# ajzhai/PEANUT

Measured on AMD Instinct MI355X. Metric: maps/sec for 480x480x(4+N_cat) prediction fwd, batch 32, higher is better.
Workload: dtype f32; 1 GPU; 480x480, 14-channel (4+10) partial maps -> 6-class prediction forward (PSPNet R50-V1c-D8), batch 32 per GPU, seeded random-init weights; survey_config=2, global_batch=32, parallelism=dp1 (map shards, no data-path collective)

## Files before the change

### peanut_amd/csrc/common.h

```cpp
#pragma once
#include <hip/hip_runtime.h>
#include <stdint.h>
#include <string>

#include "persistent_plan.h"

namespace peanut {

void set_error(const std::string& msg);
int fail(int code, const std::string& msg);
void note_kernel(const char* family);
const char* noted_kernel();

#define PEANUT_HIP_CHECK(expr)                                                            \
  do {                                                                                    \
    hipError_t _e = (expr);                                                               \
    if (_e != hipSuccess)                                                                 \
      return ::peanut::fail(-3, std::string(#expr) + ": " + hipGetErrorString(_e));       \
  } while (0)

struct ConvDesc {
  int cin;
  int cout;
  int kh, kw, stride, pad, dil;
  int relu;
  int bn_tile;
  int bk;
  int cout_pad;
  const float* w_packed;
  const float* scale;
  const float* shift;
  int rs;
  const void* w_s;
  int s_planes;
  float s_alpha;
  int flush_ch;
};

struct DeferredSplit {
  bool valid;
  const float* partial;
  int split_p, ntiles, M, cout, relu;
  const float* scale;
  const float* shift;
  float alpha;
};

struct ConvArgs {
  const float* x;
  const float* x2;
  const float* res;
  float* y;
  int B, H, W;
  int c1, c2;
  int Ho, Wo;
  float* ws;
  size_t ws_floats;
  int mt_per_group;
  size_t w_group_stride;
  int ss_group_stride;
  int group_valid_rows;
  DeferredSplit* defer;
  const int* group_rows;
};

constexpr size_t kSplitKScratchFloats = (size_t)48 << 20;
constexpr size_t kSplitKSideFloats = (size_t)8 << 20;

#if defined(__HIP_DEVICE_COMPILE__)
#define PEANUT_NO_PK_F32 __attribute__((target("no-packed-fp32-ops")))
#else
#define PEANUT_NO_PK_F32
#endif

__device__ __forceinline__ float paste_value(const float* __restrict__ m, int M, const float* __restrict__ bx, int x, int y) {
#pragma clang fp contract(off)
  const float gx = ((float)x + 0.5f - bx[0]) / (bx[2] - bx[0]) * 2.f - 1.f;
  const float gy = ((float)y + 0.5f - bx[1]) / (bx[3] - bx[1]) * 2.f - 1.f;
  const float ix = ((gx + 1.f) * (float)M - 1.f) / 2.f, iy = ((gy + 1.f) * (float)M - 1.f) / 2.f;
  const float fx = floorf(ix), fy = floorf(iy);
  const int x0 = (int)fminf(fmaxf(fx, -2.f), (float)M + 1.f), y0 = (int)fminf(fmaxf(fy, -2.f), (float)M + 1.f);
  if (x0 < -1 || x0 >= M || y0 < -1 || y0 >= M) return 0.f;
  const float lx = ix - fx, ly = iy - fy;
  const float wx = 1.f - lx, wy = 1.f - ly;
  auto at = [&](int yy, int xx) -> float {
    return ((unsigned)yy < (unsigned)M && (unsigned)xx < (unsigned)M) ? m[yy * M + xx] : 0.f;
  };
  return at(y0, x0) * wy * wx + at(y0, x0 + 1) * wy * lx + at(y0 + 1, x0) * ly * wx + at(y0 + 1, x0 + 1) * ly * lx;
}

inline int conv_out_dim(int n, int k, int s, int p, int d) { return (n + 2 * p - d * (k - 1) - 1) / s + 1; }

void conv_pick_tiles(int cin_pad, int cout, int* bn_tile, int* bk, bool pointwise = false);
size_t conv_packed_floats(int cin_pad, int cout, int kh, int kw, int bn_tile);
void pack_conv_weights(const float* w_oihw, int cout, int cin_real, int cin_pad, int kh, int kw,
                       int bn_tile, int bk, float* out);
int launch_conv(const ConvDesc& d, const ConvArgs& a, hipStream_t stream);

enum ConvKernelId {
  CONV_K_INVALID,
  CONV_K_GEMM_RS,
  CONV_K_CONV_RS,
  CONV_K_GEMM_SKINNY,
  CONV_K_PW_256X256P,
  CONV_K_PW_ARES,
  CONV_K_PW_256X256,
  CONV_K_PW_256X128P,
  CONV_K_PW_256X128,
  CONV_K_PW_TILE,
  CONV_K_PATCH,
  CONV_K_PATCH_NCHW,
  CONV_K_IGEMM,
};
struct ConvRoute {
  ConvKernelId id;
  int bm, bn, bk;
  int planes;
  int stride;
  int pack_bn;
  int G;
  PersistentPlan plan;
  int code;
  const char* error;
};
struct ConvKParams;
ConvRoute conv_route(const ConvDesc& d, const ConvArgs& a, ConvKParams* params = nullptr);
ConvRoute conv_route_patch_nchw();
const char* conv_kernel_family(const ConvRoute& r);
int device_cus();
bool conv_pw_enabled();
bool conv_pw_uses_256(int cout, long long M, int mt_per_group, int bn_tile, int cin);
int conv_pw_256_min_k();
bool conv_pw_uses_256w(int cout, long long M, int mt_per_group, int bn_tile, int cin, int flush_ktiles);
bool conv_pw_narrow_tiles(int cin, int cout, long long M, int bn_tile, int mt_per_group);
bool conv_pw_uses_256p(int cout, long long M, int mt_per_group, int bn_tile, int cin, int flush_ktiles, long long in_pixels = 0);
bool gemm_skinny_takes(const ConvKParams& p, int bn_tile, size_t ws_floats);
bool conv_pw_uses_256wp(int cout, long long M, int stride, int mt_per_group, int bn_tile, int c1, int c2, int flush_ktiles);
bool conv_pw_uses_ares(int cin, int cout, long long M, int stride, bool two_source, int flush_ktiles, int bn_tile);

bool conv_patch_eligible(const ConvDesc& d, const ConvArgs& a);
bool conv_patch_nchw_eligible(const ConvDesc& d, int B, int Ho, int Wo, int creal);
int launch_conv_patch_nchw(const ConvDesc& d, const float* x_nchw, int creal, float* y, int B, int H, int W, int Ho, int Wo, hipStream_t stream);

void wino_geometry(int B, int H, int W, int dil, int* th, int* tw, long long* n_tiles, long long* m_pad, int gran = 128, int m = 4);
void wino_transform_weights(const float* w_oihw, int cout, int cin, float* out, int m = 4);
int launch_wino_input(const float* x, float* V, int B, int H, int W, int C, int dil, hipStream_t s, int gran = 128, int m = 4, long long m_pad_total = 0,
                      const DeferredSplit* df = nullptr);
bool wino_input_accepts_deferred(int B, int H, int W, int C, int dil, int gran, int m);
long long wino_deferred_count();
int launch_wino_output(const float* Mb, const float* scale, const float* shift, const float* res, float* y,
                       int B, int H, int W, int C, int dil, int relu, hipStream_t s, int gran = 128, int m = 4, long long m_pad_total = 0);

bool gemm_rs_uses_256(int cout, long long M, int mt_per_group, int bn_tile, int cin);
bool gemm_rs_uses_64(int cout, long long M, int bn_tile, int cin);
size_t sx_packed_bytes(int cin_pad, int cout, int bn_tile, int planes);
void pack_weights_sx(const float* w, int cout, int cin_real, int cin_pad, int bn_tile, int planes, float wscale, void* out);
float sx_pack_scale(const float* w, size_t n, int planes);
size_t sx_conv_packed_bytes(int cin_pad, int cout, int kh, int kw, int bn_tile, int planes);
void pack_weights_sx_conv(const float* w_oihw, int cout, int cin_real, int cin_pad, int kh, int kw, int bn_tile, int planes,
                          float wscale, void* out);

int launch_nchw_to_nhwc_pad(const float* x, float* y, int B, int C, int H, int W, int Cpad, hipStream_t s);
int launch_maxpool3x3s2(const float* x, float* y, int B, int H, int W, int C, int Ho, int Wo, hipStream_t s);
int launch_ppm_pool(const float* x, float* out, int B, int H, int W, int C, const int* scales, int nscales,
                    hipStream_t s, int scale_rows = 0);
size_t ppm_pool_scratch_floats(int B, int H, int C, const int* scales, int nscales);
int launch_ppm_pool2(const float* x, float* scratch, float* out, int B, int H, int W, int C, const int* scales,
                     int nscales, hipStream_t s, int scale_rows = 0);
int launch_ppm_upsample_concat(const float* table, float* out, int B, int H, int W, int Cp, const int* scales,
                               int nscales, int align_corners, hipStream_t s);
int launch_ppm_conv_term(const float* Q, float* R, int B, int H, int W, int C, const int* scales, int nscales,
                         int align_corners, hipStream_t s, int scale_rows = 0);
int launch_upsample_logits(const float* lo, float* out, int B, int h, int w, int K, int H, int W,
                           int align_corners, int sigmoid, hipStream_t s);

}
```

### peanut_amd/csrc/conv_common.h

```cpp
#pragma once
#include <stdlib.h>

#include <atomic>

#include "common.h"
#include "options.h"

namespace peanut {

typedef float f32x16 __attribute__((ext_vector_type(16)));
typedef float f32x4 __attribute__((ext_vector_type(4)));

__device__ __forceinline__ float relu_keep_nan(float v) { return v < 0.f ? 0.f : v; }
__device__ __forceinline__ f32x4 relu_keep_nan(f32x4 v) {
  return f32x4{relu_keep_nan(v.x), relu_keep_nan(v.y), relu_keep_nan(v.z), relu_keep_nan(v.w)};
}

struct ConvKParams {
  const float* x;
  const float* x2;
  const float* w;
  const float* scale;
  const float* shift;
  const float* res;
  const float* zeros;
  float* y;
  int H, W, c1, c2, Ho, Wo, cout;
  int kw, ntaps, stride, pad, dil, relu;
  int M, nkt, ntiles, HoWo;
  int n_full, n_sp, split_p;
  float* partial;
  int mt_per_group;
  long long w_group_stride;
  int ss_group_stride;
  int mtiles;
  int nchunk;
  int res_prefetch;
  float alpha;
  int ares_pbn;
  int phase_shift;
  int sk_units, sk_maxp, sk_g, sk_q;
  int pack_bn;
  int group_valid;
  int p_order;
  float* dump;
  int stagger;
  int flush;
  DeferredSplit* defer;
  const int* group_rows;
};

template <int I>
struct IC { static constexpr int value = I; };
template <int N, int I = 0, class F>
__device__ __forceinline__ void static_for(F&& f) {
  if constexpr (I < N) {
    f(IC<I>{});
    static_for<N, I + 1>(f);
  }
}

struct KIter {
  int tap, ky, kx, cbase;
  const float* wtile;
};


const float* zero_page();
int launch_conv_pw(const ConvKParams& p, const ConvRoute& r, float* ws, size_t ws_floats, hipStream_t stream);
int launch_gemm_skinny(const ConvKParams& p, float* ws, size_t ws_floats, hipStream_t stream);
int launch_conv_pw_ares(const ConvKParams& p, int bn_tile, hipStream_t stream);
int launch_conv_pw256p(const ConvKParams& p, const ConvRoute& r, float* ws, hipStream_t stream);
int launch_conv_pw256wp(const ConvKParams& p, const ConvRoute& r, float* ws, hipStream_t stream);
int launch_conv_patch(const ConvKParams& p, const ConvDesc& d, int B, hipStream_t stream);
int launch_gemm_rs(const ConvKParams& p, const ConvRoute& r, int bn_tile, float* ws, size_t ws_floats, hipStream_t stream);
int launch_conv_rs(const ConvKParams& p, int bn_tile, int planes, float* ws, size_t ws_floats, hipStream_t stream);
int launch_conv_igemm(const ConvKParams& p, int bn_tile, int bk, float* ws, size_t ws_floats, hipStream_t stream);


struct Work { int mt, nt, kt0, kt1, item; };

__host__ __device__ __forceinline__ int sk_owner(long long U, int G, long long u) {
  int w = (int)(u * G / U);
  while (w + 1 < G && U * (w + 1) / G <= u) ++w;
  while (w > 0 && U * w / G > u) --w;
  return w;
}

__device__ __forceinline__ void tile_to_mn(const ConvKParams& p, int tile, int* mt_out, int* nt_out) {
  int mt, nt;
  if (p.nchunk > 0 && p.ntiles > p.nchunk) {
    const int full = p.ntiles / p.nchunk, rem = p.ntiles - full * p.nchunk;
    const int per_chunk = p.mtiles * p.nchunk;
    if (tile < full * per_chunk) {
      const int c = tile / per_chunk, r = tile - c * per_chunk;
      mt = r / p.nchunk;
      nt = c * p.nchunk + (r - mt * p.nchunk);
    } else {
      const int r = tile - full * per_chunk;
      mt = r / rem;
      nt = full * p.nchunk + (r - mt * rem);
    }
  } else {
    mt = tile / p.ntiles;
    nt = tile - mt * p.ntiles;
  }
  *mt_out = mt;
  *nt_out = nt;
}

__device__ __forceinline__ Work decode_work(const ConvKParams& p) {
  const int G = gridDim.x, bid = blockIdx.x;
  const int q = G >> 3, r = G & 7, xcd = bid & 7, local = bid >> 3;
  const int sq = p.n_sp >> 3, sr = p.n_sp & 7;
  const int sp_x = sq + (xcd < sr), sp_before = xcd * sq + (xcd < sr ? xcd : sr);
  const int chunk_before = xcd * q + (xcd < r ? xcd : r);
  Work w;
  int tile;
  if (local < sp_x) {
    const int s = sp_before + local;
    const int j = s / p.split_p, part = s - j * p.split_p;
    tile = p.n_full + j;
    w.item = s;
    w.kt0 = (int)((long long)part * p.nkt / p.split_p);
    w.kt1 = (int)((long long)(part + 1) * p.nkt / p.split_p);
  } else {
    tile = (chunk_before - sp_before) + (local - sp_x);
    w.item = -1;
    w.kt0 = 0;
    w.kt1 = p.nkt;
  }
  tile_to_mn(p, tile, &w.mt, &w.nt);
  return w;
}

constexpr int kResPrefetchRows = 8;
struct ResPrefetch { f32x4 v[kResPrefetchRows]; bool on; };

template <int BM, int BN, int EP, int NT>
__device__ __forceinline__ ResPrefetch conv_res_prefetch(const ConvKParams& p, const Work& wk, int m0, int n0) {
  constexpr int NV = BN / 4, ROWS_PER_PASS = NT / NV, ER = BM / EP;
  const int tid = threadIdx.x;
  const int c4 = (tid % NV) * 4, r0 = tid / NV, n = n0 + c4;
  ResPrefetch r;
  r.on = p.res_prefetch && p.res && wk.item < 0 && (p.cout & 3) == 0 && n < p.cout;
  if (r.on) {
#pragma unroll
    for (int i = 0; i < kResPrefetchRows; ++i) {
      const int row = r0 + i * ROWS_PER_PASS, m = m0 + row;
      r.v[i] = (row < ER && m < p.M) ? *reinterpret_cast<const f32x4*>(p.res + (size_t)m * p.cout + n) : f32x4{0.f, 0.f, 0.f, 0.f};
    }
  }
  return r;
}

template <int BM, int BN, int WM, int WN, int EP, int NT = 256, int MI = 0, int NI = 0>
__device__ __forceinline__ void conv_epilogue(const ConvKParams& p, const Work& wk, f32x16 (&acc)[MI][NI], float* smem,
                                              int m0, int n0, const ResPrefetch* early = nullptr) {
  constexpr int TM = BM / WM, TN = BN / WN;
  constexpr int CS = BN + 4, ER = BM / EP;
  static_assert(MI == TM / 32 && NI == TN / 32, "accumulator shape");
  const int tid = threadIdx.x;
  const int lane = tid & 63, wave = tid >> 6;
  const int wm = wave / WN, wn = wave % WN;
  const int li = lane & 31, hi = lane >> 5;
  constexpr int NV = BN / 4;
  constexpr int ROWS_PER_PASS = NT / NV;
  const int c4 = (tid % NV) * 4, r0 = tid / NV;
  const int n = n0 + c4;
  const int ss_off = (p.mt_per_group && p.ss_group_stride) ? (wk.mt / p.mt_per_group) * p.ss_group_stride : 0;
  const f32x4 sc = *reinterpret_cast<const f32x4*>(p.scale + ss_off + n) * p.alpha;
  const f32x4 sh = *reinterpret_cast<const f32x4*>(p.shift + ss_off + n);
  const bool vec_ok = (p.cout & 3) == 0;
  constexpr int PRE = kResPrefetchRows;
  const ResPrefetch rp = early ? *early : conv_res_prefetch<BM, BN, EP, NT>(p, wk, m0, n0);
  const f32x4 (&rpre)[PRE] = rp.v;
  const bool pre = rp.on;
#pragma unroll
  for (int ep = 0; ep < EP; ++ep) {
    if (EP == 1 || wm == ep) {
#pragma unroll
      for (int t = 0; t < MI; ++t)
#pragma unroll
        for (int u = 0; u < NI; ++u)
#pragma unroll
          for (int r = 0; r < 16; ++r) {
            const int row = wm * TM + t * 32 + (r & 3) + 8 * (r >> 2) + 4 * hi - ep * ER;
            smem[row * CS + wn * TN + u * 32 + li] = acc[t][u][r];
          }
    }
    __syncthreads();
    if (wk.item >= 0) {
      float* dst = p.partial + (size_t)wk.item * (BM * BN) + (size_t)ep * ER * BN;
      for (int row = r0; row < ER; row += ROWS_PER_PASS)
        *reinterpret_cast<f32x4*>(dst + row * BN + c4) = *reinterpret_cast<const f32x4*>(smem + row * CS + c4);
    } else {
      int row_first = r0;
      if (pre && ep == 0) {
#pragma unroll
        for (int i = 0; i < PRE; ++i) {
          const int row = r0 + i * ROWS_PER_PASS, m = m0 + row;
          if (row < ER && m < p.M) {
            f32x4 v = *reinterpret_cast<const f32x4*>(smem + row * CS + c4);
            v = v * sc + sh;
            v += rpre[i];
            if (p.relu) v = relu_keep_nan(v);
            const size_t o = (size_t)m * p.cout + n;
            *reinterpret_cast<f32x4*>(p.y + o) = v;
          }
        }
        row_first = r0 + PRE * ROWS_PER_PASS;
      }
#pragma unroll 4
      for (int row = row_first; row < ER; row += ROWS_PER_PASS) {
        const int m = m0 + ep * ER + row;
        if (m >= p.M) break;
        f32x4 v = *reinterpret_cast<const f32x4*>(smem + row * CS + c4);
        v = v * sc + sh;
        const size_t o = (size_t)m * p.cout + n;
        if (vec_ok) {
          if (n < p.cout) {
            if (p.res) v += *reinterpret_cast<const f32x4*>(p.res + o);
            if (p.relu) v = relu_keep_nan(v);
            *reinterpret_cast<f32x4*>(p.y + o) = v;
// ... 174 lines not shown
```

### peanut_amd/csrc/conv_route.hip

```cpp
#include "common.h"
#include "conv_common.h"
#include "rs_common.h"

namespace peanut {

int device_cus() {
  static std::atomic<int> cached[SlotCache::kMaxDevices];
  int dev = 0;
  if (hipGetDevice(&dev) != hipSuccess || dev < 0) return 0;
  const bool in_cache = dev < SlotCache::kMaxDevices;
  int cus = in_cache ? cached[dev].load(std::memory_order_relaxed) : 0;
  if (cus == 0) {
    if (hipDeviceGetAttribute(&cus, hipDeviceAttributeMultiprocessorCount, dev) != hipSuccess) return 0;
    if (in_cache) cached[dev].store(cus, std::memory_order_relaxed);
  }
  return cus;
}

namespace {

ConvRoute route_of(ConvKernelId id, int bm = 0, int bn = 0, int bk = 0) {
  ConvRoute r{};
  r.id = id; r.bm = bm; r.bn = bn; r.bk = bk;
  return r;
}
ConvRoute no_route(int code, const char* why) {
  ConvRoute r{};
  r.id = CONV_K_INVALID; r.code = code; r.error = why;
  return r;
}

ConvRoute route_pw(const ConvKParams& p, int bn_tile, size_t ws_floats) {
  if (gemm_skinny_takes(p, bn_tile, ws_floats)) return route_of(CONV_K_GEMM_SKINNY);
  const bool streamk = opt(OPT_PW256P_STREAMK) != 0;
  if (conv_pw_uses_256wp(p.cout, p.M, p.stride, p.mt_per_group, bn_tile, p.c1, p.c2, p.flush)) {
    const int cus = device_cus();
    if (cus < 8) return no_route(-3, "conv_pw256wp: no current device");
    ConvRoute r = route_of(CONV_K_PW_256X256P, 256, 256, 32);
    r.G = cus - cus % 8;
    r.plan = plan_persistent((p.M / 256) * (p.cout / 256), r.G, p.nkt, kPersistent256x256, streamk, ws_floats);
    if (r.plan.fits) return r;
  }
  if (conv_pw_uses_ares(p.c1, p.cout, p.M, p.stride, p.c2 != 0, p.flush, bn_tile)) return route_of(CONV_K_PW_ARES, 128, 128, 32);
  if (conv_pw_uses_256w(p.cout, p.M, p.mt_per_group, bn_tile, p.c1 + p.c2, p.flush)) return route_of(CONV_K_PW_256X256, 256, 256, 32);
  if (conv_pw_uses_256p(p.cout, p.M, p.mt_per_group, bn_tile, p.c1 + p.c2, p.flush, (long long)(p.M / p.HoWo) * p.H * p.W) && !(p.flush && p.res)) {
    const int cus = device_cus();
    if (cus < 8) return no_route(-3, "conv_pw256p: no current device");
    ConvRoute r = route_of(CONV_K_PW_256X128P, 256, 128, 32);
    r.G = cus - cus % 8;
    r.plan = plan_persistent(((p.M + 255) / 256) * p.ntiles, r.G, p.nkt, p.flush ? kPersistent256x128Flush : kPersistent256x128, streamk, ws_floats);
    if (r.plan.fits || !r.plan.scratch_ok) return r;
  }
  if (conv_pw_uses_256(p.cout, p.M, p.mt_per_group, bn_tile, p.c1 + p.c2)) return route_of(CONV_K_PW_256X128, 256, 128, 32);
  if (conv_pw_narrow_tiles(p.c1 + p.c2, p.cout, p.M, bn_tile, p.mt_per_group)) {
    ConvRoute r = route_of(CONV_K_PW_TILE, 128, 64, 32);
    r.pack_bn = 128;
    return r;
  }
  if (bn_tile != 128 && bn_tile != 64 && bn_tile != 32) return no_route(-2, "launch_conv_pw: unsupported tile configuration");
  return route_of(CONV_K_PW_TILE, 128, bn_tile, 32);
}

}

ConvRoute conv_route(const ConvDesc& d, const ConvArgs& a, ConvKParams* params) {
  if (a.c1 + a.c2 != d.cin) return no_route(-2, "launch_conv: c1 + c2 != cin");
  const bool rs_fallback = d.rs == 1 && a.c2 != 0 && d.stride != 1;
  const bool emulated = d.rs && !rs_fallback;
  const int kgran = emulated ? 16 : d.bk;
  if (a.c1 % kgran != 0 || (a.c2 % kgran) != 0) return no_route(-2, "launch_conv: channel split not a multiple of the k-tile");
  ConvKParams local;
  ConvKParams& p = params ? *params : local;
  p = ConvKParams{};
  p.x = a.x; p.x2 = a.x2 ? a.x2 : a.x; p.w = d.w_packed; p.scale = d.scale; p.shift = d.shift;
  p.res = a.res; p.y = a.y;
  p.H = a.H; p.W = a.W; p.c1 = a.c1; p.c2 = a.c2; p.Ho = a.Ho; p.Wo = a.Wo; p.cout = d.cout;
  p.kw = d.kw; p.ntaps = d.kh * d.kw; p.stride = d.stride; p.pad = d.pad; p.dil = d.dil; p.relu = d.relu;
  p.HoWo = a.Ho * a.Wo;
  const long long M = (long long)a.B * p.HoWo;
  if (M <= 0 || M > 0x7fffffffLL || (long long)a.B * a.H * a.W > 0x7fffffffLL)
    return no_route(-2, "launch_conv: problem size out of range");
  p.M = (int)M;
  p.nkt = (d.cin / d.bk) * p.ntaps;
  p.ntiles = d.cout_pad / d.bn_tile;
  p.n_full = 0; p.n_sp = 0; p.split_p = 1; p.partial = nullptr;
  p.alpha = 1.f;
  p.flush = emulated ? 0 : d.flush_ch / d.bk;
  p.mt_per_group = a.mt_per_group; p.w_group_stride = (long long)a.w_group_stride; p.ss_group_stride = a.ss_group_stride;
  p.group_valid = a.mt_per_group ? a.group_valid_rows : 0;
  p.defer = a.defer;
  p.group_rows = a.mt_per_group ? a.group_rows : nullptr;
  if (emulated) {
    p.w = static_cast<const float*>(d.w_s);
    p.nkt = (d.cin / 16) * p.ntaps;
    p.alpha = d.s_alpha;
    ConvRoute r = route_of(CONV_K_CONV_RS, 128, d.bn_tile, 16);
    if (d.rs != 2) {
      const int cin = p.c1 + p.c2;
      if (gemm_rs_uses_64(p.cout, p.M, d.bn_tile, cin)) r = route_of(CONV_K_GEMM_RS, 64, 64, 16);
      else if (gemm_rs_uses_256(p.cout, p.M, p.mt_per_group, d.bn_tile, cin)) r = route_of(CONV_K_GEMM_RS, 256, 256, 16);
      else r = route_of(CONV_K_GEMM_RS, 128, d.bn_tile == 128 ? 128 : 64, 16);
    }
    r.planes = d.s_planes;
    return r;
  }
  if (d.bk == 32 && p.ntaps == 1 && p.pad == 0 && p.c1 % 32 == 0 && p.c2 % 32 == 0 && (p.c2 == 0 || p.stride == 1) && conv_pw_enabled())
    return route_pw(p, d.bn_tile, a.ws ? a.ws_floats : 0);
  if (conv_patch_eligible(d, a)) {
    ConvRoute r = route_of(CONV_K_PATCH, 0, d.cout, d.cin);
    r.stride = d.stride;
    return r;
  }
  if ((d.bk != 32 && d.bk != 16) || (d.bn_tile != 128 && d.bn_tile != 64 && d.bn_tile != 32))
    return no_route(-2, "launch_conv: unsupported tile configuration");
  return route_of(CONV_K_IGEMM, 128, d.bn_tile, d.bk);
}

int launch_conv(const ConvDesc& d, const ConvArgs& a, hipStream_t stream) {
  ConvKParams p;
  const ConvRoute r = conv_route(d, a, &p);
  if (r.id == CONV_K_INVALID) return fail(r.code, r.error);
  p.zeros = zero_page();
  if (!p.zeros) return fail(-3, "launch_conv: zero page allocation failed");
  if (a.defer) a.defer->valid = false;
  if ((r.id == CONV_K_GEMM_RS || r.id == CONV_K_CONV_RS) && !d.w_s) return fail(-2, "launch_conv: register-split layer without pre-split weights");
  note_kernel(conv_kernel_family(r));
  switch (r.id) {
    case CONV_K_GEMM_RS: return launch_gemm_rs(p, r, d.bn_tile, a.ws, a.ws_floats, stream);
    case CONV_K_CONV_RS: return launch_conv_rs(p, d.bn_tile, d.s_planes, a.ws, a.ws_floats, stream);
    case CONV_K_GEMM_SKINNY: return launch_gemm_skinny(p, a.ws, a.ws_floats, stream);
    case CONV_K_PW_256X256P: return launch_conv_pw256wp(p, r, a.ws, stream);
    case CONV_K_PW_ARES: return launch_conv_pw_ares(p, d.bn_tile, stream);
    case CONV_K_PW_256X128P: return launch_conv_pw256p(p, r, a.ws, stream);
    case CONV_K_PW_256X256:
    case CONV_K_PW_256X128:
    case CONV_K_PW_TILE: return launch_conv_pw(p, r, a.ws, a.ws_floats, stream);
    case CONV_K_PATCH: return launch_conv_patch(p, d, a.B, stream);
    case CONV_K_IGEMM: return launch_conv_igemm(p, d.bn_tile, d.bk, a.ws, a.ws_floats, stream);
    case CONV_K_PATCH_NCHW:
    case CONV_K_INVALID: break;
  }
  return fail(-2, "launch_conv: no kernel");
}

ConvRoute conv_route_patch_nchw() {
  ConvRoute r = route_of(CONV_K_PATCH_NCHW, 0, 32, 16);
  r.stride = 2;
  return r;
}

const char* conv_kernel_family(const ConvRoute& r) {
  const int ni = r.bn == 128 ? 0 : (r.bn == 64 ? 1 : 2);
  const int kind = r.planes - RS_BF16X3;
  switch (r.id) {
    case CONV_K_INVALID: break;
    case CONV_K_IGEMM: {
      static const char* const names[2][3] = {{"conv_igemm_128x128x32", "conv_igemm_128x64x32", "conv_igemm_128x32x32"},
                                              {"conv_igemm_128x128x16", "conv_igemm_128x64x16", "conv_igemm_128x32x16"}};
      return names[r.bk == 32 ? 0 : 1][ni];
    }
    case CONV_K_CONV_RS: {
      static const char* const names[3][3] = {{"conv_rs3_128x128", "conv_rs3_128x64", "conv_rs3_128x32"},
                                              {"conv_rs6_128x128", "conv_rs6_128x64", "conv_rs6_128x32"},
                                              {"conv_rs3h_128x128", "conv_rs3h_128x64", "conv_rs3h_128x32"}};
      return kind < 0 || kind > 2 ? "conv_rs?" : names[kind][ni];
    }
    case CONV_K_GEMM_RS: {
      static const char* const names[3][4] = {{"gemm_rs3_64x64", "gemm_rs3_256x256", "gemm_rs3_128x128", "gemm_rs3_128x64"},
                                              {"gemm_rs6_64x64", "gemm_rs6_256x256", "gemm_rs6_128x128", "gemm_rs6_128x64"},
                                              {"gemm_rs3h_64x64", "gemm_rs3h_256x256", "gemm_rs3h_128x128", "gemm_rs3h_128x64"}};
      return kind < 0 || kind > 2 ? "gemm_rs?" : names[kind][r.bm == 64 ? 0 : (r.bm == 256 ? 1 : (r.bn == 128 ? 2 : 3))];
    }
    case CONV_K_GEMM_SKINNY: return "gemm_skinny";
    case CONV_K_PW_256X256P: return "conv_pw_glds_256x256p";
    case CONV_K_PW_ARES: return "conv_pw_ares_128x128";
    case CONV_K_PW_256X256: return "conv_pw_glds_256x256";
    case CONV_K_PW_256X128P: return "conv_pw_glds_256x128p";
    case CONV_K_PW_256X128: return "conv_pw_glds_256x128";
    case CONV_K_PW_TILE: return ni == 0 ? "conv_pw_glds_128x128" : (ni == 1 ? "conv_pw_glds_128x64" : "conv_pw_glds_128x32");
    case CONV_K_PATCH:
      if (r.bk == 32) return r.bn == 64 ? "conv_patch_32x64s1" : "conv_patch_32x32s1";
      return r.stride == 1 ? "conv_patch_16x32s1" : "conv_patch_16x32s2";
    case CONV_K_PATCH_NCHW: return "conv_patch_nchw_16x32s2";
  }
  return "none";
}

}
```

### peanut_amd/csrc/options.h

```cpp
#pragma once
#include <stdlib.h>
#include <string.h>

#include <string>

namespace peanut {

enum OptionId {
  OPT_PW_GLDS, OPT_PW256_MINK, OPT_PW256_MINTILES, OPT_PW256_PHASE, OPT_PW256_SKIP_PAD, OPT_PW256W_MINK, OPT_PW256W_MINTILES, OPT_PW256P_MINK, OPT_PW256P_MINTILES, OPT_PW256P_FLUSH, OPT_PW256P_ORDER, OPT_PW256P_STREAMK, OPT_PW256WP_MINK, OPT_PW256WP_MINTILES, OPT_PW256WP_NPRE, OPT_PW256WP_STAGGER, OPT_PW_ARES, OPT_PW_SKINNY,
  OPT_PW_ARES_MINUNITS, OPT_PATCH_MINTILES, OPT_STEM_NCHW, OPT_BN64_MAXK, OPT_PW_BN64_MAXK, OPT_PW64_MAXTILES, OPT_FP32_BK, OPT_NCHUNK, OPT_RES_PREFETCH, OPT_SPLIT_MODEL,
  OPT_RS_CONV, OPT_RS_BN64_MAXK, OPT_RS256_MINK, OPT_RS256_MINTILES, OPT_RS64_MAXK, OPT_RS64_MAXTILES,
  OPT_WINO_M, OPT_WINO_HEAD_M, OPT_WINO6_MAXDIL, OPT_WINO5_MINDIL, OPT_WINO_FLUSH_CH, OPT_WINO_MIN_CIN, OPT_WINO_NARROW_MINPIX, OPT_WINO_SMALL_MAXWG, OPT_DEFER_SPLITK,
  OPT_PPM_OVERLAP, OPT_PPM_GROUPED, OPT_PPM_TERM_ROWS, OPT_PPM_GROUP_ROWS, OPT_RCNN_WINO_M, OPT_RCNN_STEM_S2D, OPT_RCNN_RPN_FUSED, OPT_RCNN_FPN_OVERLAP, OPT_RCNN_RANK_SORT, OPT_RCNN_TOPK_SLICE, OPT_RCNN_NMS_LEVELS, OPT_FMM_LOCAL32, OPT_FMM_MAX_PASSES, OPT_FMM_BLOCKED, OPT_FMM_INNER,
  OPT_DEBUG_POISON_ALLOC,
  OPT_COUNT
};

struct OptionInfo {
  const char* key;
  long long def;
  bool upload_time;
  const char* help;
};

inline const OptionInfo* option_table() {
  static const OptionInfo t[OPT_COUNT] = {
      {"pw_glds", 1, false, "fp32 1x1 convs / grouped GEMMs on the LDS-DMA kernels of conv_pw.hip (0: conv_igemm)"},
      {"pw256_mink", 1024, false, "fewest input channels for the 256 x 128 three-stage kernel"},
      {"pw256_mintiles", 256, false, "fewest 256 x 128 tiles for that kernel"},
      {"pw256_phase", 1, false, "the two waves of a SIMD request their LDS-DMA pieces half an iteration apart"},
      {"pw256_skip_pad", 1, false, "256 x 128 kernel, grouped GEMMs: waves whose rows are all group padding issue no MFMAs (0: compute the zero rows)"},
      {"pw256w_mink", 768, false, "fewest input channels for the 256 x 256 two-stage kernel (0: off)"},
      {"pw256w_mintiles", 1536, false, "fewest 256 x 256 tiles for that kernel"},
      {"pw256p_mink", 512, false, "fewest input channels for the persistent 256 x 128 kernel (conv_pw256p.hip; 0: off)"},
      {"pw256p_mintiles", 512, false, "fewest 256 x 128 tiles for that kernel"},
      {"pw256p_flush", 512, false, "most input channels of a Winograd position GEMM (two-level accumulation) that runs on the persistent kernel (0: none)"},
      {"pw256p_order", 1, false, "persistent 256 x 128 kernel: 1 = the workgroups of an XCD walk its run of tiles side by side (neighbours share operand panels in L2), 0 = one contiguous run per workgroup"},
      {"pw256p_streamk", 1, false, "persistent 256 x 128 kernel: the tail tiles' k-tiles as one stream in equal runs per workgroup (0: every tail tile cut into the same number of parts)"},
      {"pw256wp_mink", 512, false, "fewest input channels for the persistent 256 x 256 kernel (conv_pw256wp.hip; 0: off)"},
      {"pw256wp_mintiles", 768, false, "fewest 256 x 256 tiles for that kernel"},
      {"pw256wp_npre", 0, false, "persistent 256 x 256 kernel: accumulator blocks per in-place epilogue group (2 or 4; 0 = two with a residual, four without)"},
      {"pw256wp_stagger", 0, false, "persistent 256 x 256 kernel: spread of the workgroups' start times in sleeps of ~3.4 us (their tile boundaries -- 512 KiB of epilogue traffic per CU -- then fall at different times)"},
      {"pw_ares", 1, false, "K = 128 / 256 pointwise layers on the persistent A-resident kernel (conv_pw_ares.hip)"},
      {"pw_skinny", 1, false, "grouped pointwise launches with at most 64 data rows per group (the PSP pyramid's per-scale convs and Q tables at batch 1) on the skinny weight-streaming kernel (gemm_skinny.hip: 6 KiB of LDS, fits next to any other kernel; 0: the MFMA kernels on 128-row padded tiles)"},
      {"pw_ares_minunits", 512, false, "fewest (m-tile, n-tile) units for that kernel"},
      {"patch_mintiles", 1024, false, "3x3 convs of 16 / 32 input channels on the persistent LDS-patch kernel (conv_patch.hip) from this many 8 x 16 output tiles (0: off)"},
      {"stem_nchw", 1, false, "prediction forward: the first stem conv reads the NCHW input itself (conv_patch.hip, NCHW variant) instead of a layout pass + NHWC conv (fp32 mode, when the patch kernel takes the layer)"},
      {"bn64_maxk", 256, true, "128 x 64 tiles for layers with at most this many input channels"},
      {"pw_bn64_maxk", 128, true, "pointwise layers / Winograd position GEMMs: weights PACKED 64 wide up to this many input channels (wider layers: 128-wide packing, 64-wide tiles chosen per shape)"},
      {"pw64_maxtiles", 512, false, "a 128-wide-packed pointwise layer with at most bn64_maxk input channels runs 128 x 64 tiles while its 128 x 128 tiling has fewer tiles than this (two per CU)"},
      {"fp32_bk", 0, true, "16: force 16-channel k-tiles in conv_igemm (experiment)"},
      {"nchunk", 8, false, "n-tiles per chunk of the tile order (0: n fastest over all n-tiles)"},
      {"res_prefetch", 1, false, "request the first residual rows before the last k-tile's MFMAs"},
      {"split_model", 1, false, "tail split-K plan counts CUs (1) or resident slots (0)"},
      {"rs_conv", 1, true, "emulated modes: non-pointwise convs on conv_rs.hip (0: fp32 MFMA kernel)"},
      {"rs_bn64_maxk", 128, true, "emulated modes: 128 x 64 tiles up to this many input channels"},
      {"rs256_mink", 512, false, "emulated modes: fewest input channels for the 256 x 256 kernel"},
      {"rs256_mintiles", 256, false, "emulated modes: fewest 256 x 256 tiles for it"},
      {"rs64_maxk", 512, false, "emulated modes: 64 x 64 tiles up to this many input channels"},
      {"rs64_maxtiles", 128, false, "emulated modes: ... and below this many 128-row tiles"},
      {"wino_m", 0, true, "4 / 5 / 6: force one Winograd form on every eligible layer (0: policy)"},
      {"wino_head_m", 0, true, "4 / 5 / 6: Winograd form of the PSP bottleneck (0: policy)"},
      {"wino6_maxdil", 4, true, "largest dilation that gets an F(6x6) form"},
      {"wino5_mindil", 4, true, "smallest dilation that also gets an F(5x5) form (0: none)"},
      {"wino_flush_ch", 64, true, "channels per partial sum of the position GEMMs' two-level accumulation (0: off)"},
      {"wino_min_cin", 0, true, "fewest input channels of a Winograd layer (0: the planner's policy)"},
      {"wino_narrow_minpix", 20000, false, "layers under 128 channels take their Winograd form from this many input pixels on (round 6: 100 000 -> 20 000 -- with the small-problem transforms one 720 x 720 map's layer1 conv2, 32 400 pixels, gains 5 us per layer as F(6x6); profiles/r9e)"},
      {"wino_small_maxwg", 1024, false, "Winograd transforms: launches with fewer workgroups than this of the one-thread-per-tile kernels take the small-problem variants (a workgroup per tile and 64-channel slice, a thread per line, through LDS; bit-identical; 0: never)"},
      {"defer_splitk", 1, false, "a Bottleneck conv1 whose every tile is split along k leaves its partial tiles unsummed and conv2's (small-problem) Winograd input transform sums them: one launch fewer per block at batch 1, bit-identical (0: every conv runs its own reduce); read when a (B, H, W) plan is built"},
      {"ppm_overlap", -1, false, "pyramid branch of the PSP head on a side stream: 0 / 1, -1 = by size"},
      {"ppm_grouped", -1, false, "per-scale PSP GEMMs as one grouped launch: 0 / 1, -1 = by size"},
      {"ppm_term_rows", 1, false, "folded pyramid term: one wave per output row, no barrier in the row loop (0: the workgroup-wide two-phase kernel)"},
      {"ppm_group_rows", 0, false, "pyramid pooling, row pass: rows added up per workgroup (1..5; 0 = by size: as many as still leave ~768 workgroups)"},
      {"rcnn_wino_m", 0, true, "detector front end: 4 / 5 / 6 pins one Winograd form (0: per shape)"},
      {"rcnn_stem_s2d", 1, true, "detector stem 7x7 stride 2 as a space-to-depth 4x4 conv"},
      {"rcnn_rpn_fused", 1, false, "detector: the RPN head on all five pyramid levels as one chain (five input transforms, ONE grouped Winograd GEMM, five output transforms, one objectness and one anchor-delta GEMM over all levels' rows: 12 launches instead of 25); read when a (B, H, W) plan is built"},
      {"rcnn_fpn_overlap", 0, false, "detector: the FPN output convs of p5, p4, p3 on a side stream next to the lateral / top-down chain that ends in p2's (round 5 experiment, bit-identical; measured SLOWER at batch 1, 5.70 against 5.61 ms per frame, profiles/r8: off); read when a (B, H, W) plan is built"},
      {"rcnn_rank_sort", 1, false, "detector: the RPN candidates of an image are ordered by counting the larger keys (n / 64 workgroups) instead of one workgroup's bitonic sort (round 5; same order: the keys are distinct)"},
      {"rcnn_topk_slice", 20480, false, "detector: objectness logits per workgroup of the per-level top-k (a level is cut into up to 8 ranges whose k largest are merged by counting; 0: one workgroup per level, round 4)"},
      {"rcnn_nms_levels", 1, false, "detector: the proposal NMS level by level (five 16 x 16-word suppression blocks and five scans per image side by side, post-NMS top-k by counting) instead of one score-sorted list per image (round 5; same proposals)"},
      {"fmm_local32", 1, false, "goal solver: single-precision local solve inside a tile"},
      {"fmm_max_passes", 24, false, "goal solver: hard ceiling of the second-order ordering passes; they stop as soon as a pass changes nothing (6-10 passes on the agent's 960 x 960 map; peanut_goal_converged reports whether they reached their fixed point)"},
      {"fmm_blocked", 1, false, "goal solver: a wave relaxes its 8 x 8 block of the tile to convergence between workgroup barriers (round 5; 0: one Jacobi sweep of the whole tile per barrier pair)"},
      {"fmm_inner", 48, false, "goal solver: iterations a wave spends on its block before it publishes it (blocked rounds)"},
      {"debug_poison_alloc", 0, false, "test switch: every device allocation the library makes for itself (workspace arenas, conv / Winograd / split-K scratch, the detector's and the goal solver's buffers, the map projection's arrays, uploaded weights before their copy) is filled with 0xFF bytes straight after hipMalloc -- fp32 / fp64 read NaN, int reads -1, 64-bit keys all ones -- so a kernel that reads a slot nothing wrote shows up as a changed result (tests/test_workspace_gpu.py); 0: allocations stay as the allocator returns them, no extra call"},
  };
  return t;
}

struct Options {
  long long v[OPT_COUNT];
};

inline int option_index(const char* key) {
  if (!key) return -1;
  std::string k(key);
  for (auto& c : k) c = (char)((c >= 'A' && c <= 'Z') ? c - 'A' + 'a' : c);
  if (k.rfind("peanut_", 0) == 0) k = k.substr(7);
  const OptionInfo* t = option_table();
  for (int i = 0; i < OPT_COUNT; ++i)
    if (k == t[i].key) return i;
  return -1;
}

inline Options& default_options() {
  static Options d = [] {
    Options o;
    const OptionInfo* t = option_table();
    for (int i = 0; i < OPT_COUNT; ++i) {
      o.v[i] = t[i].def;
      std::string env = "PEANUT_";
      for (const char* c = t[i].key; *c; ++c) env += (char)((*c >= 'a' && *c <= 'z') ? *c - 'a' + 'A' : *c);
      const char* e = getenv(env.c_str());
      if (e && *e) o.v[i] = atoll(e);
    }
    return o;
  }();
  return d;
}

inline const Options*& active_options_ptr() {
  static thread_local const Options* p = nullptr;
  return p;
}

inline long long opt(OptionId id) {
  const Options* a = active_options_ptr();
  return (a ? a : &default_options())->v[id];
}

struct OptionScope {
  const Options* saved;
  explicit OptionScope(const Options* o) : saved(active_options_ptr()) { active_options_ptr() = o; }
  ~OptionScope() { active_options_ptr() = saved; }
  OptionScope(const OptionScope&) = delete;
  OptionScope& operator=(const OptionScope&) = delete;
};

}
```

Before: 898.7 maps/s.

## Add persistent weights-resident kernel for layer1 short-K narrow-N pointwise convs

Adds a persistent pointwise-conv kernel that keeps the whole weight matrix (at most 64 KiB) resident in LDS. It streams 128-row activation tiles through a multi-slot global_load_lds ring and overlaps the previous tile's epilogue (scale/shift, residual, ReLU, stores) with the current tile's MFMAs. Routing sends layer1-style K=64->N=64/256 and K=256->N=64 pointwise layers and position GEMMs to it ahead of the A-resident kernel. The aim is to stop re-fetching weights and to hide epilogue traffic for these memory-bound layers. The hand-tuned vmcnt counts and ring depth are fragile, and only one workgroup runs per CU.

```diff
diff --git a/peanut_amd/csrc/common.h b/peanut_amd/csrc/common.h
--- a/peanut_amd/csrc/common.h
+++ b/peanut_amd/csrc/common.h
@@ -103,6 +103,7 @@
   CONV_K_CONV_RS,
   CONV_K_GEMM_SKINNY,
   CONV_K_PW_256X256P,
+  CONV_K_PW_WRES,
   CONV_K_PW_ARES,
   CONV_K_PW_256X256,
   CONV_K_PW_256X128P,
@@ -136,6 +137,7 @@
 bool conv_pw_uses_256p(int cout, long long M, int mt_per_group, int bn_tile, int cin, int flush_ktiles, long long in_pixels = 0);
 bool gemm_skinny_takes(const ConvKParams& p, int bn_tile, size_t ws_floats);
 bool conv_pw_uses_256wp(int cout, long long M, int stride, int mt_per_group, int bn_tile, int c1, int c2, int flush_ktiles);
+bool conv_pw_uses_wres(int c1, int c2, int cout, int cout_pad, long long M, int stride, int flush_ktiles, int bn_tile);
 bool conv_pw_uses_ares(int cin, int cout, long long M, int stride, bool two_source, int flush_ktiles, int bn_tile);
 
 bool conv_patch_eligible(const ConvDesc& d, const ConvArgs& a);
diff --git a/peanut_amd/csrc/conv_common.h b/peanut_amd/csrc/conv_common.h
--- a/peanut_amd/csrc/conv_common.h
+++ b/peanut_amd/csrc/conv_common.h
@@ -70,6 +70,7 @@
 int launch_conv_pw(const ConvKParams& p, const ConvRoute& r, float* ws, size_t ws_floats, hipStream_t stream);
 int launch_gemm_skinny(const ConvKParams& p, float* ws, size_t ws_floats, hipStream_t stream);
 int launch_conv_pw_ares(const ConvKParams& p, int bn_tile, hipStream_t stream);
+int launch_conv_pw_wres(const ConvKParams& p, int bn_tile, hipStream_t stream);
 int launch_conv_pw256p(const ConvKParams& p, const ConvRoute& r, float* ws, hipStream_t stream);
 int launch_conv_pw256wp(const ConvKParams& p, const ConvRoute& r, float* ws, hipStream_t stream);
 int launch_conv_patch(const ConvKParams& p, const ConvDesc& d, int B, hipStream_t stream);
diff --git a/peanut_amd/csrc/conv_pw_wres.hip b/peanut_amd/csrc/conv_pw_wres.hip
--- /dev/null
+++ b/peanut_amd/csrc/conv_pw_wres.hip
@@ -0,0 +1,295 @@
+#include <stdlib.h>
+
+#include "common.h"
+#include "conv_common.h"
+
+namespace peanut {
+
+namespace {
+
+typedef const __attribute__((address_space(1))) void* gptr_t;
+typedef __attribute__((address_space(3))) void* lptr_t;
+
+constexpr int wres_depth(int ch, int chr, int max_slots) {
+  int d = 1;
+  while (d + 2 <= max_slots && ch + d * (chr + 2 + ch) <= 60) ++d;
+  return d;
+}
+
+template <int NK, int NQ, bool FLUSH, bool RES>
+struct WresCfg {
+  static constexpr int BK = 32, K = NK * BK, N = NQ * 64, SLICE = 128 * BK;
+  static constexpr int WFLOATS = N * K;
+  static constexpr int CH = 16 / NK, CHR = RES ? CH : 0;
+  static constexpr int IT = NQ * NK;
+  static constexpr int MAX_SLOTS = ((160 * 1024 / 4 - WFLOATS) / SLICE) < 6 ? ((160 * 1024 / 4 - WFLOATS) / SLICE) : 6;
+  static constexpr int D = NQ == 1 ? wres_depth(CH, CHR, MAX_SLOTS) : 2 * NK, R = NQ == 1 ? D + 1 : D + NK;
+  static constexpr int NS = NQ == 1 ? CH + (D - 1) * (CHR + 2 + CH) : 63, NH = NQ == 1 ? 2 * (D - 1) : 63;
+  static constexpr int W_PIECES = N * NK / 64;
+  static_assert(NS <= 63 && R >= 2 && R <= MAX_SLOTS && 16 % NK == 0 && (NK & (NK - 1)) == 0, "ring / chunk shape");
+  static_assert(NQ == 1 || (2 * NQ - 3) * 16 >= 63, "NQ > 1: more stores than the counter holds between a request and its first read");
+  static_assert(!FLUSH || NK == 2, "two-level accumulation: K = 64 only");
+};
+
+template <int NK, int NQ, bool FLUSH, bool RES>
+__global__ __launch_bounds__(512) void conv_pw_wres_kernel(const ConvKParams p) {
+  using C = WresCfg<NK, NQ, FLUSH, RES>;
+  constexpr int BK = C::BK, K = C::K, N = C::N, SLICE = C::SLICE, CH = C::CH, D = C::D, R = C::R;
+  __shared__ __attribute__((aligned(1024))) float smem[C::WFLOATS + R * SLICE];
+  float* const ring = smem + C::WFLOATS;
+
+  const int tid = threadIdx.x, lane = tid & 63;
+  const int wave = __builtin_amdgcn_readfirstlane(tid >> 6);
+  const int lr = lane >> 3, lp = lane & 7;
+  const int wm = wave >> 1, wn = wave & 1;
+  const int li = lane & 31, hi = lane >> 5;
+
+  const int G = gridDim.x, bid = blockIdx.x;
+  const int lw = (G & 7) ? bid : (bid & 7) * (G >> 3) + (bid >> 3);
+  const int T = p.mtiles;
+  const int per = T / G, extra = T - per * G;
+  const int t0 = lw * per + (lw < extra ? lw : extra);
+  const int ntl = per + (lw < extra ? 1 : 0);
+  if (ntl == 0) return;
+  const int S = ntl * NK;
+
+  unsigned a_off[2];
+#pragma unroll
+  for (int j = 0; j < 2; ++j) {
+    const int r = (wave * 2 + j) * 8 + lr;
+    a_off[j] = r * K + (lp ^ ((r >> 1) & 7)) * 4;
+  }
+  auto dma_a = [&](int s, int slot) {
+    const int sc = s < S ? s : S - 1;
+    const int t = sc / NK, kt = sc - t * NK;
+    const float* base = p.x + (size_t)(t0 + t) * (128 * K) + kt * BK;
+#pragma unroll
+    for (int j = 0; j < 2; ++j)
+      __builtin_amdgcn_global_load_lds((gptr_t)(base + a_off[j]), (lptr_t)(ring + slot * SLICE + (wave * 2 + j) * 256), 16, 0, 0);
+  };
+  const int pbn = p.ares_pbn;
+  auto load_weights = [&](int g) {
+    const float* wg = p.w + (size_t)g * p.w_group_stride;
+#pragma unroll
+    for (int j = 0; j < C::W_PIECES; ++j) {
+      const int pi = wave * C::W_PIECES + j;
+      const int kt = pi / (N / 8), r = (pi - kt * (N / 8)) * 8 + lr;
+      const int c = lp ^ ((r >> 1) & 7);
+      const float* src = wg + (r / pbn) * (NK * pbn * BK) + kt * (pbn * BK) + (r % pbn) * BK + c * 4;
+      __builtin_amdgcn_global_load_lds((gptr_t)src, (lptr_t)(smem + pi * 256), 16, 0, 0);
+    }
+  };
+
+  const int swz = (li >> 1) & 7;
+  int sw[4];
+#pragma unroll
+  for (int ks = 0; ks < 4; ++ks) sw[ks] = ((ks * 2 + hi) ^ swz) * 4;
+  const int a_row = (wm * 32 + li) * BK;
+  const int b_row = (wn * 32 + li) * BK;
+
+  f32x16 acc, prev;
+#pragma unroll
+  for (int r = 0; r < 16; ++r) { acc[r] = 0.f; prev[r] = 0.f; }
+
+  const unsigned lane_el = (unsigned)(wm * 32 + 4 * hi) * N + wn * 32 + li;
+  const float alpha = p.alpha;
+  const bool relu = p.relu != 0;
+  const int mtpg = p.mt_per_group;
+  float sca[NQ], shv[NQ];
+  int g_w = mtpg ? t0 / mtpg : 0, g_ss = -1;
+  auto load_ss = [&](int t) {
+    const int g = (mtpg && p.ss_group_stride) ? t / mtpg : 0;
+    if (g == g_ss) return;
+    g_ss = g;
+#pragma unroll
+    for (int q = 0; q < NQ; ++q) {
+      sca[q] = p.scale[g * p.ss_group_stride + q * 64 + wn * 32 + li] * alpha;
+      shv[q] = p.shift[g * p.ss_group_stride + q * 64 + wn * 32 + li];
+    }
+  };
+  float resv[16], held[16];
+#pragma unroll
+  for (int i = 0; i < 16; ++i) { resv[i] = 0.f; held[i] = 0.f; }
+#define WRES_EL(r) ((unsigned)((8 * ((r) >> 2) + ((r) & 3)) * N))
+#define WRES_RES_LOADS(t, q, r0, n)                                                       \
+  {                                                                                       \
+    const float* const res_unit = p.res + (size_t)(t) * (128 * N) + (q) * 64;             \
+    _Pragma("unroll") for (int i = (r0); i < (r0) + (n); ++i) resv[i] = res_unit[lane_el + WRES_EL(i)]; \
+  }
+#define WRES_FINISH(q, r0, n)                                                             \
+  _Pragma("unroll") for (int i = (r0); i < (r0) + (n); ++i) {                             \
+    float v = prev[i] * sca[q] + shv[q];                                                  \
+    asm("" : "+v"(v));       \
+    if constexpr (RES) { v += resv[i]; asm("" : "+v"(v)); }                               \
+    if (relu) v = relu_keep_nan(v);                                                       \
+    held[i] = v;                                                                          \
+  }
+#define WRES_STORES(t, q, r0, n)                                                          \
+  {                                                                                       \
+    float* const y_unit = p.y + (size_t)(t) * (128 * N) + (q) * 64;                       \
+    _Pragma("unroll") for (int i = (r0); i < (r0) + (n); ++i) y_unit[lane_el + WRES_EL(i)] = held[i]; \
+  }
+#define WRES_MFMAS(cur_a, cur_b)                                                          \
+  {                                                                                       \
+    f32x4 af[4], bf[4];                                                                   \
+    _Pragma("unroll") for (int g4 = 0; g4 < 4; ++g4) {                                    \
+      af[g4] = *reinterpret_cast<const f32x4*>((cur_a) + a_row + sw[g4]);                 \
+      bf[g4] = *reinterpret_cast<const f32x4*>((cur_b) + b_row + sw[g4]);                 \
+    }                                                                                     \
+    _Pragma("unroll") for (int g4 = 0; g4 < 4; ++g4)                                      \
+      _Pragma("unroll") for (int kk = 0; kk < 4; ++kk) acc = __builtin_amdgcn_mfma_f32_32x32x2f32(af[g4][kk], bf[g4][kk], acc, 0, 0, 0); \
+  }
+#define WRES_UNIT_DONE()                                                                  \
+  _Pragma("unroll") for (int r = 0; r < 16; ++r) {                                        \
+    prev[r] = FLUSH ? acc[r] + 0.f : acc[r];                                              \
+    acc[r] = 0.f;                                                                         \
+  }
+
+  if constexpr (NQ > 1) load_ss(t0);
+  load_weights(g_w);
+#pragma unroll
+  for (int s = 0; s < D; ++s) dma_a(s, s);
+  asm volatile("s_waitcnt vmcnt(0)" ::: "memory");
+  __builtin_amdgcn_s_barrier();
+  asm volatile("" ::: "memory");
+
+  int s_it = 0, slot_t = 0, slot_f = D;
+  auto run_tile = [&](const int ti, auto vc) {
+    constexpr int V = decltype(vc)::value;
+    const int t = t0 + ti;
+    if (NQ == 1 && mtpg && t / mtpg != g_w) {
+      g_w = t / mtpg;
+      load_weights(g_w);
+      asm volatile("s_waitcnt vmcnt(0)" ::: "memory");
+      __builtin_amdgcn_s_barrier();
+      asm volatile("" ::: "memory");
+    }
+    if constexpr (V > 0 && NQ == 1) load_ss(t - 1);
+
+    if constexpr (NQ == 1) {
+      static_for<NK>([&](auto kc) {
+        constexpr int kt = decltype(kc)::value;
+        const float* const cur_a = ring + ((slot_t + kt) % R) * SLICE;
+        const float* const cur_b = smem + kt * (N * BK);
+        if constexpr (RES && V > 0) { WRES_RES_LOADS(t - 1, 0, kt * CH, CH) }
+        __builtin_amdgcn_sched_barrier(0);
+        dma_a(ti * NK + kt + D, slot_f);
+        slot_f = slot_f + 1 == R ? 0 : slot_f + 1;
+        __builtin_amdgcn_sched_barrier(0);
+        WRES_MFMAS(cur_a, cur_b)
+        __builtin_amdgcn_sched_barrier(0);
+        if constexpr (V > 0) {
+          WRES_FINISH(0, kt * CH, CH)
+          WRES_STORES(t - 1, 0, kt * CH, CH)
+        }
+        __builtin_amdgcn_sched_barrier(0);
+        if (s_it >= NK + D - 1) { asm volatile("s_waitcnt vmcnt(%0)" ::"n"(C::NS) : "memory"); }
+        else { asm volatile("s_waitcnt vmcnt(%0)" ::"n"(C::NH) : "memory"); }
+        asm volatile("s_waitcnt lgkmcnt(0)" ::: "memory");
+        __builtin_amdgcn_s_barrier();
+        asm volatile("" ::: "memory");
+        ++s_it;
+      });
+      WRES_UNIT_DONE()
+    } else {
+      static_for<NQ>([&](auto qc) {
+        constexpr int q = decltype(qc)::value;
+        constexpr bool has_prev = V > 0 || q > 0, has_held = V > 0 || q > 1;
+        if constexpr (RES && has_prev) {
+          if constexpr (q > 0) { WRES_RES_LOADS(t, q - 1, 0, 16) }
+          else { WRES_RES_LOADS(t - 1, NQ - 1, 0, 16) }
+        }
+        __builtin_amdgcn_sched_barrier(0);
+        if constexpr (q == 0) {
+#pragma unroll
+          for (int kt = 0; kt < NK; ++kt) {
+            dma_a(ti * NK + kt + D, slot_f);
+            slot_f = slot_f + 1 == R ? 0 : slot_f + 1;
+          }
+        }
+        __builtin_amdgcn_sched_barrier(0);
+        if constexpr (has_held) {
+          if constexpr (q > 1) { WRES_STORES(t, q - 2, 0, 16) }
+          else { WRES_STORES(t - 1, NQ - 2 + q, 0, 16) }
+        }
+        __builtin_amdgcn_sched_barrier(0);
+#pragma unroll
+        for (int kt = 0; kt < NK; ++kt) {
+          const float* const cur_a = ring + ((slot_t + kt) % R) * SLICE;
+          const float* const cur_b = smem + kt * (N * BK) + q * (64 * BK);
+          WRES_MFMAS(cur_a, cur_b)
+        }
+        __builtin_amdgcn_sched_barrier(0);
+        if constexpr (has_prev) { WRES_FINISH((q + NQ - 1) % NQ, 0, 16) }
+        if constexpr (q == NQ - 1) {
+          asm volatile("s_waitcnt vmcnt(%0)" ::"n"(C::NS) : "memory");
+          asm volatile("s_waitcnt lgkmcnt(0)" ::: "memory");
+          __builtin_amdgcn_s_barrier();
+          asm volatile("" ::: "memory");
+        }
+        WRES_UNIT_DONE()
+      });
+    }
+    slot_t = (slot_t + NK) % R;
+  };
+  run_tile(0, IC<0>{});
+  for (int ti = 1; ti < ntl; ++ti) run_tile(ti, IC<1>{});
+
+  {
+    const int t = t0 + ntl - 1;
+    if constexpr (NQ == 1) load_ss(t);
+    else { WRES_STORES(t, NQ - 2, 0, 16) }
+    if constexpr (RES) { WRES_RES_LOADS(t, NQ - 1, 0, 16) }
+    WRES_FINISH(NQ - 1, 0, 16)
+    WRES_STORES(t, NQ - 1, 0, 16)
+  }
+  asm volatile("s_waitcnt vmcnt(0)" ::: "memory");
+#undef WRES_EL
+#undef WRES_RES_LOADS
+#undef WRES_FINISH
+#undef WRES_STORES
+#undef WRES_MFMAS
+#undef WRES_UNIT_DONE
+}
+
+template <int NK, int NQ, bool FLUSH, bool RES>
+int launch_wres_t(const ConvKParams& p, int G, hipStream_t stream) {
+  hipLaunchKernelGGL((conv_pw_wres_kernel<NK, NQ, FLUSH, RES>), dim3((unsigned)G), dim3(512), 0, stream, p);
+  hipError_t e = hipGetLastError();
+  if (e != hipSuccess) return fail(-3, std::string("conv_pw_wres launch: ") + hipGetErrorString(e));
+  return 0;
+}
+
+template <int NK, int NQ, bool FLUSH>
+int launch_wres_r(const ConvKParams& p, int G, hipStream_t stream) {
+  return p.res ? launch_wres_t<NK, NQ, FLUSH, true>(p, G, stream) : launch_wres_t<NK, NQ, FLUSH, false>(p, G, stream);
+}
+
+}
+
+bool conv_pw_uses_wres(int c1, int c2, int cout, int cout_pad, long long M, int stride, int flush_ktiles, int bn_tile) {
+  if (opt(OPT_PW_WRES) == 0 || c2 != 0 || stride != 1 || M % 128 != 0 || cout != cout_pad) return false;
+  if (bn_tile != 64 && bn_tile != 128) return false;
+  const bool shape = (c1 == 64 && (cout == 64 || cout == 256)) || (c1 == 256 && cout == 64);
+  if (!shape || (long long)c1 * cout * 4 > 64 * 1024) return false;
+  if (flush_ktiles != 0 && !(flush_ktiles == 2 && c1 == 64 && cout == 64)) return false;
+  if (M * (c1 > cout ? c1 : cout) * 4 >= (1LL << 32)) return false;
+  return M / 128 >= opt(OPT_PW_WRES_MINTILES);
+}
+
+int launch_conv_pw_wres(const ConvKParams& p0, int bn_tile, hipStream_t stream) {
+  ConvKParams p = p0;
+  p.ares_pbn = bn_tile;
+  p.mtiles = p.M / 128;
+  p.ntiles = 1;
+  const int cus = device_cus();
+  if (cus < 1) return fail(-3, "conv_pw_wres: no current device");
+  int G = cus >= 8 ? cus - cus % 8 : cus;
+  const long long cap = opt(OPT_PW_WRES_GRID);
+  if (cap > 0 && cap < G) G = (int)cap;
+  if (p.c1 == 256) return launch_wres_r<8, 1, false>(p, G, stream);
+  if (p.cout == 256) return launch_wres_r<2, 4, false>(p, G, stream);
+  return p.flush ? launch_wres_r<2, 1, true>(p, G, stream) : launch_wres_r<2, 1, false>(p, G, stream);
+}
+
+}
diff --git a/peanut_amd/csrc/conv_route.hip b/peanut_amd/csrc/conv_route.hip
--- a/peanut_amd/csrc/conv_route.hip
+++ b/peanut_amd/csrc/conv_route.hip
@@ -41,6 +41,7 @@
     r.plan = plan_persistent((p.M / 256) * (p.cout / 256), r.G, p.nkt, kPersistent256x256, streamk, ws_floats);
     if (r.plan.fits) return r;
   }
+  if (conv_pw_uses_wres(p.c1, p.c2, p.cout, p.ntiles * bn_tile, p.M, p.stride, p.flush, bn_tile)) return route_of(CONV_K_PW_WRES, 128, p.cout, 32);
   if (conv_pw_uses_ares(p.c1, p.cout, p.M, p.stride, p.c2 != 0, p.flush, bn_tile)) return route_of(CONV_K_PW_ARES, 128, 128, 32);
   if (conv_pw_uses_256w(p.cout, p.M, p.mt_per_group, bn_tile, p.c1 + p.c2, p.flush)) return route_of(CONV_K_PW_256X256, 256, 256, 32);
   if (conv_pw_uses_256p(p.cout, p.M, p.mt_per_group, bn_tile, p.c1 + p.c2, p.flush, (long long)(p.M / p.HoWo) * p.H * p.W) && !(p.flush && p.res)) {
@@ -130,6 +131,7 @@
     case CONV_K_CONV_RS: return launch_conv_rs(p, d.bn_tile, d.s_planes, a.ws, a.ws_floats, stream);
     case CONV_K_GEMM_SKINNY: return launch_gemm_skinny(p, a.ws, a.ws_floats, stream);
     case CONV_K_PW_256X256P: return launch_conv_pw256wp(p, r, a.ws, stream);
+    case CONV_K_PW_WRES: return launch_conv_pw_wres(p, d.bn_tile, stream);
     case CONV_K_PW_ARES: return launch_conv_pw_ares(p, d.bn_tile, stream);
     case CONV_K_PW_256X128P: return launch_conv_pw256p(p, r, a.ws, stream);
     case CONV_K_PW_256X256:
@@ -173,6 +175,7 @@
     }
     case CONV_K_GEMM_SKINNY: return "gemm_skinny";
     case CONV_K_PW_256X256P: return "conv_pw_glds_256x256p";
+    case CONV_K_PW_WRES: return r.bn == 64 ? "conv_pw_wres_128x64" : "conv_pw_wres_128x256";
     case CONV_K_PW_ARES: return "conv_pw_ares_128x128";
     case CONV_K_PW_256X256: return "conv_pw_glds_256x256";
     case CONV_K_PW_256X128P: return "conv_pw_glds_256x128p";
diff --git a/peanut_amd/csrc/options.h b/peanut_amd/csrc/options.h
--- a/peanut_amd/csrc/options.h
+++ b/peanut_amd/csrc/options.h
@@ -8,6 +8,7 @@
 
 enum OptionId {
   OPT_PW_GLDS, OPT_PW256_MINK, OPT_PW256_MINTILES, OPT_PW256_PHASE, OPT_PW256_SKIP_PAD, OPT_PW256W_MINK, OPT_PW256W_MINTILES, OPT_PW256P_MINK, OPT_PW256P_MINTILES, OPT_PW256P_FLUSH, OPT_PW256P_ORDER, OPT_PW256P_STREAMK, OPT_PW256WP_MINK, OPT_PW256WP_MINTILES, OPT_PW256WP_NPRE, OPT_PW256WP_STAGGER, OPT_PW_ARES, OPT_PW_SKINNY,
+  OPT_PW_WRES, OPT_PW_WRES_MINTILES, OPT_PW_WRES_GRID,
   OPT_PW_ARES_MINUNITS, OPT_PATCH_MINTILES, OPT_STEM_NCHW, OPT_BN64_MAXK, OPT_PW_BN64_MAXK, OPT_PW64_MAXTILES, OPT_FP32_BK, OPT_NCHUNK, OPT_RES_PREFETCH, OPT_SPLIT_MODEL,
   OPT_RS_CONV, OPT_RS_BN64_MAXK, OPT_RS256_MINK, OPT_RS256_MINTILES, OPT_RS64_MAXK, OPT_RS64_MAXTILES,
   OPT_WINO_M, OPT_WINO_HEAD_M, OPT_WINO6_MAXDIL, OPT_WINO5_MINDIL, OPT_WINO_FLUSH_CH, OPT_WINO_MIN_CIN, OPT_WINO_NARROW_MINPIX, OPT_WINO_SMALL_MAXWG, OPT_DEFER_SPLITK,
@@ -43,6 +44,9 @@
       {"pw256wp_stagger", 0, false, "persistent 256 x 256 kernel: spread of the workgroups' start times in sleeps of ~3.4 us (their tile boundaries -- 512 KiB of epilogue traffic per CU -- then fall at different times)"},
       {"pw_ares", 1, false, "K = 128 / 256 pointwise layers on the persistent A-resident kernel (conv_pw_ares.hip)"},
       {"pw_skinny", 1, false, "grouped pointwise launches with at most 64 data rows per group (the PSP pyramid's per-scale convs and Q tables at batch 1) on the skinny weight-streaming kernel (gemm_skinny.hip: 6 KiB of LDS, fits next to any other kernel; 0: the MFMA kernels on 128-row padded tiles)"},
+      {"pw_wres", 1, false, "layer1's short-K, narrow-N pointwise layers and position GEMMs (K = 64 -> N = 64 / 256, K = 256 -> N = 64; weights <= 64 KiB) on the persistent weights-resident kernel (conv_pw_wres.hip); 0: every layer where it went before"},
+      {"pw_wres_mintiles", 1024, false, "fewest 128-row m-tiles for that kernel (four per CU)"},
+      {"pw_wres_grid", 0, false, "weights-resident kernel: most workgroups of a launch (0 = one per CU)"},
       {"pw_ares_minunits", 512, false, "fewest (m-tile, n-tile) units for that kernel"},
       {"patch_mintiles", 1024, false, "3x3 convs of 16 / 32 input channels on the persistent LDS-patch kernel (conv_patch.hip) from this many 8 x 16 output tiles (0: off)"},
       {"stem_nchw", 1, false, "prediction forward: the first stem conv reads the NCHW input itself (conv_patch.hip, NCHW variant) instead of a layout pass + NHWC conv (fp32 mode, when the patch kernel takes the layer)"},
```

Result: no change. 903.7 maps/s, median of 6 (+0.6%).
